# DredderGun/accbpg_and_fw

Measured on AMD Instinct MI355X. Metric: D-opt iters/sec (m=2048,n=32768), higher is better.
Workload: dtype f64; 1 GPU; D_opt_design(2048,32768) abpg_gain gamma=2 fp64, one independent instance per GPU; instances=1, instances_per_gpu=1, seeds=1..1, window=transient: iterations 5..161 from x0 = 1/n, linear_gram=False

## Files before the change

### accbpg_and_fw_amd/csrc/dopt_kernels.hip

```cpp
#include <atomic>
#include <mutex>
#include <unordered_map>
#include <type_traits>

#include "internal.h"
#include "mfma_tile.hpp"

namespace accbpg {

struct GramSeg {
    int64_t row0, col0, kb, ke;
    bool dual, whole;
};
constexpr int GRAM_RMAX = 4;
template <class T>
__device__ __forceinline__ GramSeg gram_segment(const TileRC* __restrict__ tiles, int64_t kiters, int64_t it,
                                                int64_t it1) {
    const int e = (int)(it / kiters);
    const int64_t off = it - (int64_t)e * kiters;
    const TileRC tr = tiles[e];
    GramSeg g;
    if (tr.d1 < 0) {
        g.row0 = (int64_t)tr.rb * T::BM; g.col0 = (int64_t)tr.cb * T::BN;
        g.kb = off; g.ke = min(kiters, off + (it1 - it));
// ... 390 lines not shown
    const int64_t col0 = (int64_t)blockIdx.x * T::BN;
    const int lane = threadIdx.x & 63, wave = __builtin_amdgcn_readfirstlane(threadIdx.x >> 6);
    const int wm = wave / T::WAVES_N, wn = wave % T::WAVES_N;
    const int lr = lane & 15;
    double colsum[T::NI];
#pragma unroll
    for (int j = 0; j < T::NI; ++j) colsum[j] = 0.0;
    T t;
    const int nrb = (int)((m + T::BM - 1) / T::BM);
    for (int rb = 0; rb < nrb; ++rb) {
        const int64_t row0 = (int64_t)rb * T::BM;
        const int64_t Kend = min(row0 + T::BM, m);
        const int64_t ksteps = (Kend + BK - 1) / BK;
        t.zero();
        t.gload_A(W, ldw, row0, m, 0, Kend, vec_ok_w);
        t.gload_B_km(V, ldv, col0, n, 0, Kend, vec_ok_v);
        __syncthreads();
        t.sstore(lds);
        __syncthreads();
        const int64_t klast = ksteps - 1;
        {
            const int64_t k1 = min((int64_t)1, klast);
            t.gload_A(W, ldw, row0, m, k1 * BK, Kend, vec_ok_w);
            t.gload_B_km(V, ldv, col0, n, k1 * BK, Kend, vec_ok_v);
        }
        t.template read_frag<0>(lds, 0);
        int cur = 0;
#pragma unroll 1
        for (int64_t ks = 0; ks < ksteps; ++ks) {
            const int64_t k2 = min(ks + 2, klast);
            const double* st = lds + cur * T::STAGE_ELEMS;
            double* nx = lds + (cur ^ 1) * T::STAGE_ELEMS;
            const int64_t kd = ks * BK - row0;
            int mi_lo = 0;
            if (kd > 0) {
                const int64_t num = kd - 15 - 16 * wm;
                mi_lo = num > 0 ? (int)((num + 16 * T::WAVES_M - 1) / (16 * T::WAVES_M)) : 0;
            }
            t.template read_frag<1>(st, 1);
            t.template mma_frag<0>(mi_lo);
            t.template read_frag<0>(st, 2);
            t.template mma_frag<1>(mi_lo);
            t.template read_frag<1>(st, 3);
            t.sstore(nx);
            t.template mma_frag<0>(mi_lo);
            __syncthreads();
            t.gload_A(W, ldw, row0, m, k2 * BK, Kend, vec_ok_w);
            t.gload_B_km(V, ldv, col0, n, k2 * BK, Kend, vec_ok_v);
            t.template read_frag<0>(nx, 0);
            t.template mma_frag<1>(mi_lo);
            cur ^= 1;
        }
#pragma unroll
        for (int j = 0; j < T::NI; ++j) {
            double s = 0.0;
#pragma unroll
            for (int i = 0; i < T::MI; ++i)
#pragma unroll
                for (int r = 0; r < 4; ++r) s += t.acc[i][j][r] * t.acc[i][j][r];
            colsum[j] += s;
        }
    }
#pragma unroll
    for (int j = 0; j < T::NI; ++j) {
        double s = colsum[j];
        s += __shfl_xor(s, 16);
        s += __shfl_xor(s, 32);
        colsum[j] = s;
    }
    if (lane < 16) {
#pragma unroll
        for (int j = 0; j < T::NI; ++j) red[wm][wn * T::WN + 16 * j + lr] = colsum[j];
    }
    __syncthreads();
    for (int c = threadIdx.x; c < T::BN; c += NTHREADS) {
        double s = 0.0;
#pragma unroll
        for (int w = 0; w < T::WAVES_M; ++w) s += red[w][c];
        if (col0 + c < n) out[col0 + c] = sign * s;
    }
}

constexpr int COLNORM_CV = 256;

template <class T, int G, int JJ, int RUN, int NLD>
__device__ __forceinline__ void colnorm_diag_step(T& t, double* __restrict__ lds, int& cur, int wm, int64_t kdiag,
                                                  int64_t ldv, const char* next_a) {
    int nx1 = cur + 1;
    if (nx1 >= 3) nx1 -= 3;
    int nx2 = cur + 2;
    if (nx2 >= 3) nx2 -= 3;
    constexpr int J = 4 * G + JJ;
    int64_t k2 = kdiag + J + 2;
    if constexpr (J >= 14) {
        if constexpr (J == 14) t.gbase_a = next_a;
        k2 = J - 14;
    }
    constexpr int ILO_NEXT = JJ == 3 ? ((G + 1) & 3) : G;
    t.template grad_step<RUN, G, ILO_NEXT, (JJ > 0), NLD>(lds + cur * T::G_STAGE, lds + nx1 * T::G_STAGE, lds + nx2 * T::G_STAGE,
                                                          k2 * BK, k2 * BK * ldv, wm >= JJ);
    cur = nx1;
}
template <class T, int G, int RUN, int NLD>
__device__ __forceinline__ void colnorm_diag_group(T& t, double* __restrict__ lds, int& cur, int wm, int64_t kdiag,
                                                   int64_t ldv, const char* next_a) {
    colnorm_diag_step<T, G, 0, RUN, NLD>(t, lds, cur, wm, kdiag, ldv, next_a);
    colnorm_diag_step<T, G, 1, RUN, NLD>(t, lds, cur, wm, kdiag, ldv, next_a);
    colnorm_diag_step<T, G, 2, RUN, NLD>(t, lds, cur, wm, kdiag, ldv, next_a);
    colnorm_diag_step<T, G, 3, RUN, NLD>(t, lds, cur, wm, kdiag, ldv, next_a);
}

template <class T>
__device__ __forceinline__ void colnorm_phases_body(
    const double* __restrict__ W, int64_t ldw, const double* __restrict__ V, int64_t ldv, int64_t m, int64_t n,
    double* __restrict__ out, double sign) {
    extern __shared__ __attribute__((aligned(16))) double lds[];
    double* red = lds + 3 * T::G_STAGE;
    constexpr int NLD = T::G_NA + T::G_NB;
    constexpr int RUN = 4;
    static_assert(T::WAVES_N == 1 && T::MI == 4 && T::BM == 16 * BK, "diagonal groups are laid out for the 256 x 128 tile");
    const int64_t col0 = (int64_t)blockIdx.x * T::BN;
    const int lane = threadIdx.x & 63, wave = __builtin_amdgcn_readfirstlane(threadIdx.x >> 6);
    const int wm = wave / T::WAVES_N, wn = wave % T::WAVES_N;
    const int lr = lane & 15;
    double colsum[T::NI];
#pragma unroll
    for (int j = 0; j < T::NI; ++j) colsum[j] = 0.0;
    T t;
    const int nrb = (int)(m / T::BM);
    t.template glds_setup_A<RUN>(W, ldw, 0);
    t.template glds_setup_B_km<RUN>(V, ldv, col0);
    t.template glds_issue<RUN>(0, 0, lds);
    t.template glds_issue<RUN>(BK, BK * ldv, lds + T::G_STAGE);
    asm volatile("s_waitcnt vmcnt(%0)" ::"n"(NLD) : "memory");
    __builtin_amdgcn_s_barrier();
    int cur = 0;
    t.template read_frag_lo<0, 0>(lds, 0);
    t.zero();
    t.pin_acc();
    for (int rb = 0;;) {
        const int64_t kdiag = (int64_t)rb * (T::BM / BK);
        const int rbn = rb + 1 < nrb ? rb + 1 : rb;
        const char* next_a = reinterpret_cast<const char*>(W + (int64_t)rbn * T::BM * ldw);
        colnorm_diag_group<T, 0, RUN, NLD>(t, lds, cur, wm, kdiag, ldv, next_a);
        colnorm_diag_group<T, 1, RUN, NLD>(t, lds, cur, wm, kdiag, ldv, next_a);
        colnorm_diag_group<T, 2, RUN, NLD>(t, lds, cur, wm, kdiag, ldv, next_a);
        colnorm_diag_group<T, 3, RUN, NLD>(t, lds, cur, wm, kdiag, ldv, next_a);
#pragma unroll
        for (int j = 0; j < T::NI; ++j) {
            t.pin_acc_col(j);
            double s = 0.0;
#pragma unroll
            for (int i = 0; i < T::MI; ++i)
#pragma unroll
                for (int r = 0; r < 4; ++r) s += t.acc[i][j][r] * t.acc[i][j][r];
            colsum[j] += s;
            asm volatile("" : "+v"(colsum[j]));
            __builtin_amdgcn_sched_barrier(0);
        }
        if (++rb == nrb) break;
        t.zero();
        t.pin_acc();
        const int64_t krect = (int64_t)rb * (T::BM / BK);
        int64_t ks = 0;
#pragma unroll 1
        do {
            int nx1 = cur + 1;
            if (nx1 >= 3) nx1 -= 3;
            int nx2 = cur + 2;
            if (nx2 >= 3) nx2 -= 3;
            const int64_t k2 = (ks + 2) * BK;
            t.template grad_step<RUN, 0, 0, false, NLD>(lds + cur * T::G_STAGE, lds + nx1 * T::G_STAGE, lds + nx2 * T::G_STAGE,
                                                        k2, k2 * ldv, true);
            cur = nx1;
        } while (++ks < krect);
    }
    asm volatile("s_waitcnt vmcnt(0)\n\ts_waitcnt lgkmcnt(0)" ::: "memory");
#pragma unroll
    for (int j = 0; j < T::NI; ++j) {
        double s = colsum[j];
        s += __shfl_xor(s, 16);
        s += __shfl_xor(s, 32);
        colsum[j] = s;
    }
    __syncthreads();
    if (lane < 16) {
#pragma unroll
        for (int j = 0; j < T::NI; ++j) red[wm * T::BN + wn * T::WN + 16 * j + lr] = colsum[j];
    }
    __syncthreads();
    for (int c = threadIdx.x; c < T::BN; c += NTHREADS) {
        double s = 0.0;
#pragma unroll
        for (int w = 0; w < T::WAVES_M; ++w) s += red[w * T::BN + c];
        if (col0 + c < n) out[col0 + c] = sign * s;
    }
}

template <class T, int CV>
__device__ __forceinline__ void colnorm_restart_body(
    const double* __restrict__ W, int64_t ldw, const double* __restrict__ V, int64_t ldv, int64_t m, int64_t n,
    double* __restrict__ out, double sign) {
    constexpr int AB = (CV & 512) ? (CV & 15) : 0;
    extern __shared__ __attribute__((aligned(16))) double lds[];
    double* red = lds + 3 * T::G_STAGE;
    constexpr int NLD = T::G_NA + T::G_NB;
    const int64_t col0 = (int64_t)blockIdx.x * T::BN;
    const int lane = threadIdx.x & 63, wave = __builtin_amdgcn_readfirstlane(threadIdx.x >> 6);
    const int wm = wave / T::WAVES_N, wn = wave % T::WAVES_N;
    const int lr = lane & 15;
    double colsum[T::NI];
#pragma unroll
    for (int j = 0; j < T::NI; ++j) colsum[j] = 0.0;
    T t;
    const int nrb = (int)(m / T::BM);
    for (int rb = 0; rb < nrb; ++rb) {
        const int64_t row0 = (int64_t)rb * T::BM;
        const int64_t ksteps = (row0 + T::BM) / BK;
        const int64_t klast = ksteps - 1;
        t.zero();
        constexpr int RUN = (CV & 256) ? 4 : 1;
        t.template glds_setup_A<RUN>(W, ldw, row0);
        t.template glds_setup_B_km<RUN>(V, ldv, col0);
        auto issue = [&](int64_t ks, int buf) {
            t.template glds_issue<RUN>(ks * BK, ks * BK * ldv, lds + buf * T::G_STAGE);
        };
        const int64_t ks0 = (AB & 2) ? row0 / BK : 0, ks1 = (AB & 1) ? row0 / BK : ksteps;
        if (!(AB & 8) || rb == 0) {
            __builtin_amdgcn_s_barrier();
            issue(ks0, 0);
            issue(min(ks0 + 1, klast), 1);
            asm volatile("s_waitcnt vmcnt(%0)" ::"n"(NLD) : "memory");
            __builtin_amdgcn_s_barrier();
        }
        int cur = 0;
        t.template read_frag_g<0, false>(lds, 0);
        if constexpr (CV & 32) {
            constexpr int NP = T::G_NA + T::G_NB;
#pragma unroll 1
            for (int64_t ks = ks0; ks < ks1; ++ks) {
                int nx2 = cur + 2;
                if (nx2 >= 3) nx2 -= 3;
                int nx1 = cur + 1;
                if (nx1 >= 3) nx1 -= 3;
                const double* st = lds + cur * T::G_STAGE;
                const double* st1 = lds + nx1 * T::G_STAGE;
                double* nst = lds + nx2 * T::G_STAGE;
                const int64_t kd = ks * BK - row0;
                int mi_lo = 0;
                if (kd > 0) {
                    const int64_t num = kd - 15 - 16 * wm;
                    mi_lo = num > 0 ? (int)((num + 16 * T::WAVES_M - 1) / (16 * T::WAVES_M)) : 0;
                }
                const int64_t k2 = min(ks + 2, klast) * BK;
                auto group = [&](auto gtag) {
                    constexpr int g = decltype(gtag)::value;
// ... 33 lines not shown
            }
        } else {
#pragma unroll 1
        for (int64_t ks = ks0; ks < ks1; ++ks) {
            int nx2 = cur + 2;
            if (nx2 >= 3) nx2 -= 3;
            const double* st = lds + cur * T::G_STAGE;
            const int64_t kd = ks * BK - row0;
            int mi_lo = 0;
            if (kd > 0) {
                const int64_t num = kd - 15 - 16 * wm;
                mi_lo = num > 0 ? (int)((num + 16 * T::WAVES_M - 1) / (16 * T::WAVES_M)) : 0;
            }
            constexpr int NP = T::G_NA + T::G_NB;
            constexpr int P1 = (NP + 2) / 3, P2 = 2 * P1 < NP ? 2 * P1 : NP;
            static_assert(T::MI == 4, "group 0 is dealt out over four fragment rows");
            double* nst = lds + nx2 * T::G_STAGE;
            const int64_t k2 = min(ks + 2, klast) * BK;
            if constexpr (!(AB & 4)) t.template read_frag_g<1, false>(st, 1);
            __builtin_amdgcn_sched_barrier(0);
            t.template mma_row<0>(0, mi_lo);
            if constexpr (!(AB & 4)) t.template glds_issue_range<RUN>(k2, k2 * ldv, nst, 0, P1);
            t.template mma_row<0>(1, mi_lo);
            if constexpr (!(AB & 4)) t.template glds_issue_range<RUN>(k2, k2 * ldv, nst, P1, P2);
            t.template mma_row<0>(2, mi_lo);
            if constexpr (!(AB & 4)) t.template glds_issue_range<RUN>(k2, k2 * ldv, nst, P2, NP);
            t.template mma_row<0>(3, mi_lo);
            __builtin_amdgcn_sched_barrier(0);
            if constexpr (!(AB & 4)) t.template read_frag_g<0, false>(st, 2);
            __builtin_amdgcn_sched_barrier(0);
            t.template mma_frag<1>(mi_lo);
            __builtin_amdgcn_sched_barrier(0);
            if constexpr (!(AB & 4)) t.template read_frag_g<1, false>(st, 3);
            __builtin_amdgcn_sched_barrier(0);
            t.template mma_frag<0>(mi_lo);
            __builtin_amdgcn_sched_barrier(0);
            if constexpr (!(AB & 4)) {
                asm volatile("s_waitcnt vmcnt(%0)\n\ts_waitcnt lgkmcnt(0)" ::"n"(NLD) : "memory");
                __builtin_amdgcn_s_barrier();
            }
            cur = (cur + 1 == 3) ? 0 : cur + 1;
            if constexpr (!(AB & 4)) t.template read_frag_g<0, false>(lds + cur * T::G_STAGE, 0);
            __builtin_amdgcn_sched_barrier(0);
            t.template mma_frag<1>(mi_lo);
            __builtin_amdgcn_sched_barrier(0);
        }
        }
        if (!(AB & 8) || rb == nrb - 1) asm volatile("s_waitcnt vmcnt(0)\n\ts_waitcnt lgkmcnt(0)" ::: "memory");
#pragma unroll
        for (int j = 0; j < T::NI; ++j) {
            double s = 0.0;
#pragma unroll
            for (int i = 0; i < T::MI; ++i)
#pragma unroll
                for (int r = 0; r < 4; ++r) s += t.acc[i][j][r] * t.acc[i][j][r];
            colsum[j] += s;
        }
    }
#pragma unroll
    for (int j = 0; j < T::NI; ++j) {
        double s = colsum[j];
        s += __shfl_xor(s, 16);
        s += __shfl_xor(s, 32);
        colsum[j] = s;
    }
    __syncthreads();
    if (lane < 16) {
#pragma unroll
        for (int j = 0; j < T::NI; ++j) red[wm * T::BN + wn * T::WN + 16 * j + lr] = colsum[j];
    }
    __syncthreads();
    for (int c = threadIdx.x; c < T::BN; c += NTHREADS) {
        double s = 0.0;
#pragma unroll
        for (int w = 0; w < T::WAVES_M; ++w) s += red[w * T::BN + c];
        if (col0 + c < n) out[col0 + c] = sign * s;
    }
}

template <class T, int CV = 0>
__device__ __forceinline__ void colnorm_glds_body(
    const double* __restrict__ W, int64_t ldw, const double* __restrict__ V, int64_t ldv, int64_t m, int64_t n,
    double* __restrict__ out, double sign) {
    if constexpr (CV == COLNORM_CV) colnorm_phases_body<T>(W, ldw, V, ldv, m, n, out, sign);
    else colnorm_restart_body<T, CV>(W, ldw, V, ldv, m, n, out, sign);
}

template <class T, int CV = 0>
__global__ __launch_bounds__(NTHREADS, 1) void colnorm_glds_kernel(
    const double* __restrict__ W, int64_t ldw, const double* __restrict__ V, int64_t ldv, int64_t m, int64_t n,
    double* __restrict__ out, double sign) {
    colnorm_glds_body<T, CV>(W, ldw, V, ldv, m, n, out, sign);
}
template <class T>
__global__ __launch_bounds__(NTHREADS, 1) void colnorm_glds_batch_kernel(
    const BatchInst* __restrict__ bt, BatchAct act, int64_t ldw, int64_t ldv, int64_t m, int64_t n,
    double* __restrict__ outbase, int64_t ldo, double sign) {
    const int inst = act.idx[blockIdx.y];
    const BatchInst bi = bt[inst];
    colnorm_glds_body<T, COLNORM_CV>(bi.Wbuf, ldw, bi.V, ldv, m, n, outbase + (int64_t)inst * ldo, sign);
}

template <class T, int LOOP>
__device__ __forceinline__ void gemm_ops_body(const GemmOp op) {
    extern __shared__ __attribute__((aligned(16))) double lds[];
    const int64_t row0 = (int64_t)blockIdx.y * T::BM, col0 = (int64_t)blockIdx.x * T::BN;
    if (row0 >= op.M || col0 >= op.N) return;
    if (op.lower_only && col0 > row0 + T::BM - 1) return;
    const bool va = ((reinterpret_cast<uintptr_t>(op.A) & 15) == 0) && ((op.lda & 1) == 0);
    const bool vb = ((reinterpret_cast<uintptr_t>(op.B) & 15) == 0) && ((op.ldb & 1) == 0);
    T t;
    t.zero();
    int64_t ksteps = (op.K + BK - 1) / BK;
    int64_t ks0 = 0;
    if (op.tri & 1) ks0 = max((int64_t)0, col0 - op.koff) / BK;
    if (op.tri & 2) ksteps = min(ksteps, max((int64_t)0, row0 + T::BM - op.koff + BK - 1) / BK);
    if (ks0 >= ksteps) {
        t.store_C(op.C, op.ldc, row0, col0, op.M, op.N, op.alpha, op.beta, op.lower_only != 0);
        return;
    }
    if constexpr (LOOP == 0) {
        auto gload = [&](int64_t ks) {
            t.gload_A(op.A, op.lda, row0, op.M, ks * BK, op.K, va);
            if constexpr (T::BKM) t.gload_B_km(op.B, op.ldb, col0, op.N, ks * BK, op.K, vb);
            else t.gload_B_kc(op.B, op.ldb, col0, op.N, ks * BK, op.K, vb);
        };
        gload(ks0);
        t.sstore(lds);
        __syncthreads();
        int cur = 0;
        for (int64_t ks = ks0; ks < ksteps; ++ks) {
            const bool more = ks + 1 < ksteps;
            if (more) gload(ks + 1);
            t.compute(lds + cur * T::STAGE_ELEMS);
            if (more) t.sstore(lds + (cur ^ 1) * T::STAGE_ELEMS);
            __syncthreads();
            cur ^= 1;
        }
    } else {
        constexpr int D = LOOP;
        const bool inside = va && vb && row0 + T::BM <= op.M && col0 + T::BN <= op.N && ksteps * BK <= op.K;
        d2 pa[D][T::A_PASS], pb[D][T::B_PASS];
        auto sstore_from = [&](auto slot, double* __restrict__ stage) {
            constexpr int S = decltype(slot)::value;
#pragma unroll
            for (int p = 0; p < T::A_PASS; ++p) t.ra[p] = pa[S][p];
#pragma unroll
            for (int p = 0; p < T::B_PASS; ++p) t.rb[p] = pb[S][p];
            t.sstore(stage);
        };
        auto run = [&](auto guard) {
            constexpr bool GUARD = decltype(guard)::value;
            auto gload_to = [&](auto slot, int64_t ks) {
                constexpr int S = decltype(slot)::value;
                t.template gload_A<GUARD>(as_global(op.A), op.lda, row0, op.M, ks * BK, op.K, va);
                if constexpr (T::BKM) t.template gload_B_km<GUARD>(as_global(op.B), op.ldb, col0, op.N, ks * BK, op.K, vb);
                else t.template gload_B_kc<GUARD>(as_global(op.B), op.ldb, col0, op.N, ks * BK, op.K, vb);
#pragma unroll
                for (int p = 0; p < T::A_PASS; ++p) pa[S][p] = t.ra[p];
#pragma unroll
                for (int p = 0; p < T::B_PASS; ++p) pb[S][p] = t.rb[p];
            };
            static_for<0, D>([&](auto j) {
                if (ks0 + decltype(j)::value < ksteps) gload_to(j, ks0 + decltype(j)::value);
            });
            sstore_from(std::integral_constant<int, 0>{}, lds);
            if (ks0 + D < ksteps) gload_to(std::integral_constant<int, 0>{}, ks0 + D);
// ... 1843 lines not shown
    accbpg_dopt* h0 = b->inst[0];
    static bool lds_set = false;
    if (!lds_set) {
        ACC_TRY(set_lds(gram_streamk_glds_batch_kernel<T>, T::G_LDS_BYTES));
        lds_set = true;
    }
    prof_begin(h0, PROF_GRAM);
    gram_streamk_glds_batch_kernel<T><<<dim3(h0->gram_grid, act.n), NTHREADS, T::G_LDS_BYTES, b->stream>>>(
        b->table, act, h0->ldv, h0->m, h0->n, xbase, ldx, h0->tiles, h0->wg_ranges, h0->kiters, h0->gram_nslot, h0->m);
    prof_end(h0, PROF_GRAM);
    prof_begin(h0, PROF_GRAMFIX);
    gram_fixup_batch_kernel<T><<<dim3(h0->ntiles * 2 * T::MI * FIX_PJ, act.n), NTHREADS, 0, b->stream>>>(
        b->table, act, h0->tiles, h0->gram_cstart, h0->gram_contrib, h0->gram_nslot, h0->m, h0->m);
    prof_end(h0, PROF_GRAMFIX);
    ACC_HIP(hipGetLastError());
    return ACCBPG_OK;
}

int launch_cholesky_batch(accbpg_dopt_batch* b, const BatchAct& act, bool with_inverse, const double* xbase, int64_t ldx) {
    accbpg_dopt* h0 = b->inst[0];
    const int64_t m = h0->m;
    const int T = (int)((m + NB - 1) / NB);
    prof_begin(h0, PROF_CHOL);
    zero_scalars_batch_kernel<<<act.n, 512, 0, b->stream>>>(b->table, act, xbase, ldx, h0->n, T * T + 5 * T);
    const int dev = (b->device >= 0 && b->device < 64) ? b->device : 0;
    const int grid_all = h0->chol_tiles_grid * act.n;
    std::lock_guard<std::mutex> lk(g_tiles_mu);
    TilesRing& ring = g_tiles[dev];
    {
        int gmax = grid_all;
        for (int i = 0; i < TILES_RING; ++i) gmax = std::max(gmax, ring.grid[i]);
        int together = std::max(1, h0->chol_slots) / std::max(1, gmax);
        if (together > TILES_RING - 1) together = TILES_RING - 1;
        if (together < 1) together = 1;
        for (long long back = together; back <= TILES_RING && back <= ring.issued; ++back) {
            const int slot = (int)((ring.issued - back) % TILES_RING);
            if (ring.ev[slot] && ring.stream[slot] != b->stream) ACC_HIP(hipStreamWaitEvent(b->stream, ring.ev[slot], 0));
        }
    }
    chol_tiles_kernel<<<dim3(h0->chol_tiles_grid, act.n), NTHREADS, CT_LDS_BYTES, b->stream>>>(
        CholInst{}, b->chol_table[with_inverse ? 1 : 0], reinterpret_cast<const CholJob*>(h0->chol_jobs), m, m, T,
        h0->chol_spin_limit, 0, act);
    prof_end(h0, PROF_CHOL);
    ACC_HIP(hipGetLastError());
    {
        const int slot = (int)(ring.issued % TILES_RING);
        if (!ring.ev[slot]) ACC_HIP(hipEventCreateWithFlags(&ring.ev[slot], hipEventDisableTiming));
        ACC_HIP(hipEventRecord(ring.ev[slot], b->stream));
        ring.stream[slot] = b->stream;
        ring.grid[slot] = grid_all;
        ++ring.issued;
    }
    return ACCBPG_OK;
}

int launch_trtri_batch(accbpg_dopt_batch* b, const BatchAct& act) {
    accbpg_dopt* h0 = b->inst[0];
    prof_begin(h0, PROF_TRTRI);
    for (const accbpg_dopt::MergeStage& st : h0->merge_stages) {
        const int count = st.end - st.begin;
        if (count <= 0) continue;
        if (st.kind == 0) {
            dim3 grid((st.maxn + 63) / 64, (st.maxm + 63) / 64, count * act.n);
            ACC_TRY(with_gemm_loop([&](auto loop) -> int {
                gemm_ops_batch_kernel<TileSmall<true>, decltype(loop)::value><<<grid, NTHREADS, TileSmall<true>::LDS_BYTES, b->stream>>>(
                    b->ops_all, b->ops_per_inst, st.begin, count, act);
                return ACCBPG_OK;
            }));
        } else {
            int gx = (int)std::min<int64_t>(1024, ((int64_t)st.maxm / 2 + 255) / 256);
            gemm_reduce_batch_kernel<<<dim3(gx, count * act.n), 256, 0, b->stream>>>(b->red_all, b->red_per_inst, st.begin, count, act);
        }
    }
    prof_end(h0, PROF_TRTRI);
    ACC_HIP(hipGetLastError());
    return ACCBPG_OK;
}

int debug_grad_variant(accbpg_dopt* h, double* out, int var, int iters, double* ms_out) {
    using T = TileBig<true, false>;
    const bool vw = ((reinterpret_cast<uintptr_t>(h->Wbuf) & 15) == 0) && ((h->m & 1) == 0);
    if (!h->big || !h->use_glds || !vw || !h->vec_ok || h->m % 256 != 0 || h->n % 128 != 0) return ACCBPG_ERR_ARG;
    const int grid = (int)(h->n / T::BN), lds = T::G_LDS_BYTES + 4 * T::BN * 8;
    if (var != 0 && var != 3 && (var < 10 || var > 13)) return ACCBPG_ERR_ARG;
    hipEvent_t a, b;
    ACC_HIP(hipEventCreate(&a));
    if (hipEventCreate(&b) != hipSuccess) {
        hipEventDestroy(a);
        return ACCBPG_ERR_HIP;
    }
    auto launch = [&]() -> int {
#define ACC_LAUNCH_C(CC) \
    ACC_LAUNCH_LDS((colnorm_glds_kernel<T, CC>), grid, NTHREADS, lds, h->stream, h->Wbuf, h->m, h->V, h->ldv, h->m, h->n, out, -1.0)
        switch (var) {
            case 0: ACC_LAUNCH_C(COLNORM_CV); break;
            case 3: ACC_LAUNCH_C(COLNORM_CV | 512); break;
            case 10: ACC_LAUNCH_C(COLNORM_CV | 512 | 1); break;
            case 11: ACC_LAUNCH_C(COLNORM_CV | 512 | 2); break;
            case 12: ACC_LAUNCH_C(COLNORM_CV | 512 | 4); break;
            case 13: ACC_LAUNCH_C(COLNORM_CV | 512 | 8); break;
            default: return ACCBPG_ERR_ARG;
        }
#undef ACC_LAUNCH_C
        return ACCBPG_OK;
    };
    auto timed = [&]() -> int {
        ACC_TRY(launch());
        ACC_HIP(hipEventRecord(a, h->stream));
        for (int i = 0; i < iters; ++i) ACC_TRY(launch());
        ACC_HIP(hipEventRecord(b, h->stream));
        ACC_HIP(hipEventSynchronize(b));
        float ms = 0.f;
        ACC_HIP(hipEventElapsedTime(&ms, a, b));
        *ms_out = ms / iters;
        ACC_HIP(hipGetLastError());
        return ACCBPG_OK;
    };
    const int rc = timed();
    hipEventDestroy(a);
    hipEventDestroy(b);
    return rc;
}

int launch_colnorm_batch(accbpg_dopt_batch* b, const BatchAct& act, double* gbase, int64_t ldg, double sign) {
    using T = TileBig<true, false>;
    accbpg_dopt* h0 = b->inst[0];
    static bool lds_set = false;
    if (!lds_set) {
        ACC_TRY(set_lds(colnorm_glds_batch_kernel<T>, T::G_LDS_BYTES + 4 * T::BN * 8));
        lds_set = true;
    }
    prof_begin(h0, PROF_GRAD);
    colnorm_glds_batch_kernel<T><<<dim3((unsigned)(h0->n / T::BN), act.n), NTHREADS, T::G_LDS_BYTES + 4 * T::BN * 8, b->stream>>>(
        b->table, act, h0->m, h0->ldv, h0->m, h0->n, gbase, ldg, sign);
    prof_end(h0, PROF_GRAD);
    ACC_HIP(hipGetLastError());
    return ACCBPG_OK;
}

int launch_test_gemm(const double* A, int64_t lda, const double* B, int64_t ldb, double* C, int64_t ldc, int64_t M,
                     int64_t N, int64_t K, int b_kmajor, double alpha, double beta, int config, hipStream_t s) {
    GemmOp op{};
    op.A = A; op.B = B; op.C = C; op.lda = lda; op.ldb = ldb; op.ldc = ldc;
    op.M = (int)M; op.N = (int)N; op.K = (int)K; op.lower_only = 0; op.alpha = alpha; op.beta = beta;
    if (config == 1) {
        if (b_kmajor) {
            using T = TileBig<true>;
            ACC_TRY(set_lds(gemm_big_kernel<T>, T::LDS_BYTES));
            dim3 grid((unsigned)((N + T::BN - 1) / T::BN), (unsigned)((M + T::BM - 1) / T::BM));
            gemm_big_kernel<T><<<grid, NTHREADS, T::LDS_BYTES, s>>>(op);
        } else {
            using T = TileBig<false>;
            ACC_TRY(set_lds(gemm_big_kernel<T>, T::LDS_BYTES));
            dim3 grid((unsigned)((N + T::BN - 1) / T::BN), (unsigned)((M + T::BM - 1) / T::BM));
            gemm_big_kernel<T><<<grid, NTHREADS, T::LDS_BYTES, s>>>(op);
        }
    } else {
        GemmOp* d = nullptr;
        ACC_HIP(hipMalloc(&d, sizeof(GemmOp)));
        ACC_HIP(hipMemcpyAsync(d, &op, sizeof(GemmOp), hipMemcpyHostToDevice, s));
        ACC_TRY(set_lds_gemm_ops());
        int rc = launch_gemm_ops(d, 1, (int)M, (int)N, b_kmajor != 0, s);
        hipStreamSynchronize(s);
        hipFree(d);
        return rc;
    }
    ACC_HIP(hipGetLastError());
    return ACCBPG_OK;
}

int pipe_probe(int iters, int mode, double* ms_out, hipStream_t s) {
    int dev = 0;
    hipDeviceProp_t prop;
    ACC_HIP(hipGetDevice(&dev));
    ACC_HIP(hipGetDeviceProperties(&prop, dev));
    double* sink = nullptr;
    ACC_HIP(hipMalloc(&sink, 8));
    hipEvent_t a, b;
    ACC_HIP(hipEventCreate(&a));
    ACC_HIP(hipEventCreate(&b));
    pipe_probe_kernel<<<prop.multiProcessorCount, NTHREADS, 0, s>>>(iters / 10 + 1, mode, sink);
    ACC_HIP(hipEventRecord(a, s));
    pipe_probe_kernel<<<prop.multiProcessorCount, NTHREADS, 0, s>>>(iters, mode, sink);
// ... 37 lines not shown
```

### accbpg_and_fw_amd/csrc/mfma_tile.hpp

```cpp
#pragma once
#include <hip/hip_runtime.h>
#include <stdint.h>
#include <type_traits>

namespace accbpg {

typedef double d4 __attribute__((ext_vector_type(4)));
typedef double d2 __attribute__((ext_vector_type(2)));

constexpr int BK = 16;
constexpr int SK = BK + 2;
constexpr int NTHREADS = 256;

typedef const __attribute__((address_space(1))) double* gptr;
__device__ __forceinline__ gptr as_global(const double* p) { return (gptr)p; }
__device__ __forceinline__ d2 ld2(const double* p) { return *reinterpret_cast<const d2*>(p); }
__device__ __forceinline__ d2 ld2(gptr p) { return *(const __attribute__((address_space(1))) d2*)p; }

template <class P>
__device__ __forceinline__ d2 load2_guard(P p, bool row_ok, int64_t k, int64_t K, bool vec_ok) {
    d2 v;
    if (row_ok && vec_ok && k + 1 < K) {
        v = ld2(p);
    } else {
// ... 352 lines not shown
        if constexpr (BKM) {
            const double* bs = stage + G_A + (4 * kk + lq) * BN + wn * WN + lr;
#pragma unroll
            for (int j = 0; j < NI; ++j) fb[SET][j] = bs[16 * (j ^ (lq & 1))];
        } else {
            const double* bs = stage + G_A + (wn * WN + lr) * BK + koff;
#pragma unroll
            for (int j = 0; j < NI; ++j) fb[SET][j] = bs[j * 16 * BK];
        }
        if constexpr (SCALE) fx[SET] = stage[G_A + G_B + 4 * kk + lq];
    }

    template <int SET, bool SCALE, int PART>
    __device__ __forceinline__ void read_part_g(const double* __restrict__ stage, int kk) {
        static_assert(MI == 4 && NI == 8, "parts are laid out for the 64 x 128 wave tile");
        const int lane = threadIdx.x & 63, wave = __builtin_amdgcn_readfirstlane(threadIdx.x >> 6);
        const int wm = wave / WAVES_N, wn = wave % WAVES_N;
        const int lr = lane & 15, lq = lane >> 4;
        const int sw = (lr >> 1) & 7;
        const int koff = 2 * ((2 * kk + (lq >> 1)) ^ sw) + (lq & 1);
        if constexpr (PART == 0) {
            if constexpr (SCALE) fx[SET] = stage[G_A + G_B + 4 * kk + lq];
        } else if constexpr (PART == 1 || PART == 6) {
            const double* as = stage + (16 * wm + lr) * BK + koff;
            constexpr int i0 = (PART == 1) ? 0 : 2;
            fa[SET][i0] = as[i0 * 16 * WAVES_M * BK];
            fa[SET][i0 + 1] = as[(i0 + 1) * 16 * WAVES_M * BK];
        } else {
            constexpr int j0 = 2 * (PART - 2);
            if constexpr (BKM) {
                const double* bs = stage + G_A + (4 * kk + lq) * BN + wn * WN + lr;
                fb[SET][j0] = bs[16 * (j0 ^ (lq & 1))];
                fb[SET][j0 + 1] = bs[16 * ((j0 + 1) ^ (lq & 1))];
            } else {
                const double* bs = stage + G_A + (wn * WN + lr) * BK + koff;
                fb[SET][j0] = bs[j0 * 16 * BK];
                fb[SET][j0 + 1] = bs[(j0 + 1) * 16 * BK];
            }
        }
    }
    template <int SET, int I>
    __device__ __forceinline__ void scale_row() { fa[SET][I] *= fx[SET]; }
    template <int SET, int I, int P>
    __device__ __forceinline__ void mma_pair(int mi_lo = 0) {
        if (I >= mi_lo) {
            acc[I][2 * P] = __builtin_amdgcn_mfma_f64_16x16x4f64(fa[SET][I], fb[SET][2 * P], acc[I][2 * P], 0, 0, 0);
            acc[I][2 * P + 1] = __builtin_amdgcn_mfma_f64_16x16x4f64(fa[SET][I], fb[SET][2 * P + 1], acc[I][2 * P + 1], 0, 0, 0);
        }
    }

    template <int SET, int ILO>
    __device__ __forceinline__ void read_frag_lo(const double* __restrict__ stage, int kk) {
        static_assert(BKM, "the gradient product reads a k-major B image");
        const int lane = threadIdx.x & 63, wave = __builtin_amdgcn_readfirstlane(threadIdx.x >> 6);
        const int wm = wave / WAVES_N, wn = wave % WAVES_N;
        const int lr = lane & 15, lq = lane >> 4;
        const int sw = (lr >> 1) & 7;
        const int koff = 2 * ((2 * kk + (lq >> 1)) ^ sw) + (lq & 1);
        const double* as = stage + (16 * wm + lr) * BK + koff;
#pragma unroll
        for (int i = ILO; i < MI; ++i) fa[SET][i] = as[i * 16 * WAVES_M * BK];
        const double* bs = stage + G_A + (4 * kk + lq) * BN + wn * WN + lr;
#pragma unroll
        for (int j = 0; j < NI; ++j) fb[SET][j] = bs[16 * (j ^ (lq & 1))];
    }
    template <int SET, int I, int ILO, bool COND>
    __device__ __forceinline__ void mma_row_lo(bool live) {
        if constexpr (I >= ILO) {
            if (!(COND && I == ILO) || live) {
#pragma unroll
                for (int j = 0; j < NI; ++j)
                    acc[I][j] = __builtin_amdgcn_mfma_f64_16x16x4f64(fa[SET][I], fb[SET][j], acc[I][j], 0, 0, 0);
            }
        }
    }
    template <int SET, int ILO, bool COND>
    __device__ __forceinline__ void mma_frag_lo(bool live) {
        static_assert(MI == 4, "four fragment rows");
        mma_row_lo<SET, 0, ILO, COND>(live);
        mma_row_lo<SET, 1, ILO, COND>(live);
        mma_row_lo<SET, 2, ILO, COND>(live);
        mma_row_lo<SET, 3, ILO, COND>(live);
    }
    template <int RUN, int ILO, int ILO_NEXT, bool COND, int NLD>
    __device__ __forceinline__ void grad_step(const double* __restrict__ st, const double* __restrict__ st1,
                                              double* __restrict__ nst, int64_t ka, int64_t kb, bool live) {
        constexpr int NP = G_NA + G_NB;
        constexpr int P1 = (NP + 2) / 3, P2 = 2 * P1 < NP ? 2 * P1 : NP;
        static_assert(NLD == NP, "every wave retires the loads of one step per step");
        read_frag_lo<1, ILO>(st, 1);
        __builtin_amdgcn_sched_barrier(0);
        mma_row_lo<0, 0, ILO, COND>(live);
        glds_issue_range<RUN>(ka, kb, nst, 0, P1);
        mma_row_lo<0, 1, ILO, COND>(live);
        glds_issue_range<RUN>(ka, kb, nst, P1, P2);
        mma_row_lo<0, 2, ILO, COND>(live);
        glds_issue_range<RUN>(ka, kb, nst, P2, NP);
        mma_row_lo<0, 3, ILO, COND>(live);
        __builtin_amdgcn_sched_barrier(0);
        read_frag_lo<0, ILO>(st, 2);
        __builtin_amdgcn_sched_barrier(0);
        mma_frag_lo<1, ILO, COND>(live);
        __builtin_amdgcn_sched_barrier(0);
        read_frag_lo<1, ILO>(st, 3);
        __builtin_amdgcn_sched_barrier(0);
        mma_frag_lo<0, ILO, COND>(live);
        __builtin_amdgcn_sched_barrier(0);
        asm volatile("s_waitcnt vmcnt(%0)\n\ts_waitcnt lgkmcnt(0)" ::"n"(NLD) : "memory");
        __builtin_amdgcn_s_barrier();
        read_frag_lo<0, ILO_NEXT>(st1, 0);
        __builtin_amdgcn_sched_barrier(0);
        mma_frag_lo<1, ILO, COND>(live);
        __builtin_amdgcn_sched_barrier(0);
    }

    double fb2[2][NI];
    __device__ __forceinline__ void glds_setup_A_dual(const double* __restrict__ V, int64_t ldv, int64_t band0,
                                                      int64_t khalf) {
        const int lane = threadIdx.x & 63, wave = __builtin_amdgcn_readfirstlane(threadIdx.x >> 6);
        gbase_a = reinterpret_cast<const char*>(V + band0 * ldv);
#pragma unroll
        for (int p = 0; p < G_NA; ++p) {
            const int q = wave + 4 * p;
            const int row = 8 * q + (lane >> 3);
            const int c = (lane & 7) ^ ((row >> 1) & 7);
            goa[p] = (uint32_t)(((int64_t)(row & (BM / 2 - 1)) * ldv + 2 * c + ((row >= BM / 2) ? khalf : 0)) * 8);
        }
    }
    __device__ __forceinline__ void glds_issue_dual(int64_t ka, const double* __restrict__ x, int64_t khalf,
                                                    double* __restrict__ stage) const {
        const int lane = threadIdx.x & 63, wave = __builtin_amdgcn_readfirstlane(threadIdx.x >> 6);
        const char* ba = gbase_a + ka * 8;
#pragma unroll
        for (int p = 0; p < G_NA; ++p) {
            uint32_t o = goa[p];
            asm volatile("" : "+v"(o));
            glds16(reinterpret_cast<const double*>(ba + o), stage + (wave + 4 * p) * 128);
        }
        const float* sx = reinterpret_cast<const float*>(x + ka + ((lane & 32) ? khalf : 0)) + (lane & 31);
        __builtin_amdgcn_global_load_lds((const __attribute__((address_space(1))) void*)sx,
                                         (__attribute__((address_space(3))) void*)(stage + G_A + G_B), 4, 0, 0);
    }
    static constexpr int G_NLD_DUAL = G_NA + 1;
    static __device__ __forceinline__ int dual_row_block(int i2, int w) {
        return i2 ? (2 * WAVES_M - 1 - w) : w;
    }
    template <int SET>
    __device__ __forceinline__ void read_frag_dual(const double* __restrict__ stage, int kk) {
        const int lane = threadIdx.x & 63, wave = __builtin_amdgcn_readfirstlane(threadIdx.x >> 6);
        const int lr = lane & 15, lq = lane >> 4;
        const int sw = (lr >> 1) & 7;
        const int koff = 2 * ((2 * kk + (lq >> 1)) ^ sw) + (lq & 1);
#pragma unroll
        for (int i = 0; i < MI; ++i)
            fa[SET][i] = stage[((i / (MI / 2)) * (BM / 2) + 16 * dual_row_block(i % (MI / 2), wave) + lr) * BK + koff];
        const double* bs = stage + lr * BK + koff;
#pragma unroll
        for (int j = 0; j < NI; ++j) {
            fb[SET][j] = bs[j * 16 * BK];
            fb2[SET][j] = bs[(BM / 2 + j * 16) * BK];
        }
        fx[SET] = stage[G_A + G_B + 4 * kk + lq];
        fx2[SET] = stage[G_A + G_B + 16 + 4 * kk + lq];
    }
    double fx2[2];
    template <int SET>
    __device__ __forceinline__ void scale_dual() {
#pragma unroll
        for (int i = 0; i < MI; ++i) fa[SET][i] *= (i < MI / 2) ? fx[SET] : fx2[SET];
    }
    template <int SET>
    __device__ __forceinline__ void mma_dual() {
        const int wave = __builtin_amdgcn_readfirstlane(threadIdx.x >> 6);
#pragma unroll
        for (int i = 0; i < MI; ++i) {
            const int lim = dual_row_block(i % (MI / 2), wave);
#pragma unroll
            for (int j = 0; j < NI; ++j) {
                if (j > lim) break;
                acc[i][j] = __builtin_amdgcn_mfma_f64_16x16x4f64(fa[SET][i], (i < MI / 2) ? fb[SET][j] : fb2[SET][j],
                                                                 acc[i][j], 0, 0, 0);
            }
        }
    }
    __device__ __forceinline__ void store_C(double* __restrict__ C, int64_t ldc, int64_t row0, int64_t col0,
                                            int64_t M, int64_t N, double alpha, double beta, bool lower_only) const {
        const int lane = threadIdx.x & 63, wave = __builtin_amdgcn_readfirstlane(threadIdx.x >> 6);
        const int wm = wave / WAVES_N, wn = wave % WAVES_N;
        const int lr = lane & 15, lq = lane >> 4;
#pragma unroll
        for (int i = 0; i < MI; ++i)
#pragma unroll
            for (int j = 0; j < NI; ++j)
#pragma unroll
                for (int r = 0; r < 4; ++r) {
                    const int64_t row = row0 + 16 * (i * WAVES_M + wm) + lq + 4 * r;
// ... 133 lines not shown
```

Before: 64.49 iterations/s.

## Interleave fragment reads and global loads between individual MFMA pairs in colnorm

```diff
diff --git a/accbpg_and_fw_amd/csrc/dopt_kernels.hip b/accbpg_and_fw_amd/csrc/dopt_kernels.hip
--- a/accbpg_and_fw_amd/csrc/dopt_kernels.hip
+++ b/accbpg_and_fw_amd/csrc/dopt_kernels.hip
@@ -496,8 +496,11 @@
 }
 
 constexpr int COLNORM_CV = 256;
-
-template <class T, int G, int JJ, int RUN, int NLD>
+constexpr int COLNORM_BLOCK = 1024, COLNORM_OTHER_PLACEMENT = 2048, COLNORM_ABLATE = 4096, COLNORM_DIAG_BLOCK = 8192;
+constexpr bool COLNORM_PB = true;
+constexpr bool colnorm_pb(int cv) { return ((cv & COLNORM_OTHER_PLACEMENT) != 0) != COLNORM_PB; }
+
+template <class T, int G, int JJ, int RUN, int NLD, int CV>
 __device__ __forceinline__ void colnorm_diag_step(T& t, double* __restrict__ lds, int& cur, int wm, int64_t kdiag,
                                                   int64_t ldv, const char* next_a) {
     int nx1 = cur + 1;
@@ -511,20 +514,25 @@
         k2 = J - 14;
     }
     constexpr int ILO_NEXT = JJ == 3 ? ((G + 1) & 3) : G;
-    t.template grad_step<RUN, G, ILO_NEXT, (JJ > 0), NLD>(lds + cur * T::G_STAGE, lds + nx1 * T::G_STAGE, lds + nx2 * T::G_STAGE,
-                                                          k2 * BK, k2 * BK * ldv, wm >= JJ);
+    constexpr int AB = (CV & COLNORM_ABLATE) ? (CV & 7) : 0;
+    if constexpr (!(CV & (COLNORM_BLOCK | COLNORM_DIAG_BLOCK)) && T::template dealt_pairs_per_group<G, (JJ > 0)>() >= 12)
+        t.template grad_step_dealt<RUN, G, ILO_NEXT, (JJ > 0), NLD, colnorm_pb(CV), AB>(
+            lds + cur * T::G_STAGE, lds + nx1 * T::G_STAGE, lds + nx2 * T::G_STAGE, k2 * BK, k2 * BK * ldv, wm >= JJ);
+    else
+        t.template grad_step<RUN, G, ILO_NEXT, (JJ > 0), NLD, AB>(lds + cur * T::G_STAGE, lds + nx1 * T::G_STAGE, lds + nx2 * T::G_STAGE,
+                                                                  k2 * BK, k2 * BK * ldv, wm >= JJ);
     cur = nx1;
 }
-template <class T, int G, int RUN, int NLD>
+template <class T, int G, int RUN, int NLD, int CV>
 __device__ __forceinline__ void colnorm_diag_group(T& t, double* __restrict__ lds, int& cur, int wm, int64_t kdiag,
                                                    int64_t ldv, const char* next_a) {
-    colnorm_diag_step<T, G, 0, RUN, NLD>(t, lds, cur, wm, kdiag, ldv, next_a);
-    colnorm_diag_step<T, G, 1, RUN, NLD>(t, lds, cur, wm, kdiag, ldv, next_a);
-    colnorm_diag_step<T, G, 2, RUN, NLD>(t, lds, cur, wm, kdiag, ldv, next_a);
-    colnorm_diag_step<T, G, 3, RUN, NLD>(t, lds, cur, wm, kdiag, ldv, next_a);
-}
-
-template <class T>
+    colnorm_diag_step<T, G, 0, RUN, NLD, CV>(t, lds, cur, wm, kdiag, ldv, next_a);
+    colnorm_diag_step<T, G, 1, RUN, NLD, CV>(t, lds, cur, wm, kdiag, ldv, next_a);
+    colnorm_diag_step<T, G, 2, RUN, NLD, CV>(t, lds, cur, wm, kdiag, ldv, next_a);
+    colnorm_diag_step<T, G, 3, RUN, NLD, CV>(t, lds, cur, wm, kdiag, ldv, next_a);
+}
+
+template <class T, int CV>
 __device__ __forceinline__ void colnorm_phases_body(
     const double* __restrict__ W, int64_t ldw, const double* __restrict__ V, int64_t ldv, int64_t m, int64_t n,
     double* __restrict__ out, double sign) {
@@ -532,6 +540,8 @@
     double* red = lds + 3 * T::G_STAGE;
     constexpr int NLD = T::G_NA + T::G_NB;
     constexpr int RUN = 4;
+    constexpr int AB = (CV & COLNORM_ABLATE) ? (CV & 7) : 0;
+    constexpr bool PB = colnorm_pb(CV);
     static_assert(T::WAVES_N == 1 && T::MI == 4 && T::BM == 16 * BK, "diagonal groups are laid out for the 256 x 128 tile");
     const int64_t col0 = (int64_t)blockIdx.x * T::BN;
     const int lane = threadIdx.x & 63, wave = __builtin_amdgcn_readfirstlane(threadIdx.x >> 6);
@@ -550,16 +560,17 @@
     __builtin_amdgcn_s_barrier();
     int cur = 0;
     t.template read_frag_lo<0, 0>(lds, 0);
+    if constexpr (AB & 4) t.template read_frag_lo<1, 0>(lds, 1);
     t.zero();
     t.pin_acc();
     for (int rb = 0;;) {
         const int64_t kdiag = (int64_t)rb * (T::BM / BK);
         const int rbn = rb + 1 < nrb ? rb + 1 : rb;
         const char* next_a = reinterpret_cast<const char*>(W + (int64_t)rbn * T::BM * ldw);
-        colnorm_diag_group<T, 0, RUN, NLD>(t, lds, cur, wm, kdiag, ldv, next_a);
-        colnorm_diag_group<T, 1, RUN, NLD>(t, lds, cur, wm, kdiag, ldv, next_a);
-        colnorm_diag_group<T, 2, RUN, NLD>(t, lds, cur, wm, kdiag, ldv, next_a);
-        colnorm_diag_group<T, 3, RUN, NLD>(t, lds, cur, wm, kdiag, ldv, next_a);
+        colnorm_diag_group<T, 0, RUN, NLD, CV>(t, lds, cur, wm, kdiag, ldv, next_a);
+        colnorm_diag_group<T, 1, RUN, NLD, CV>(t, lds, cur, wm, kdiag, ldv, next_a);
+        colnorm_diag_group<T, 2, RUN, NLD, CV>(t, lds, cur, wm, kdiag, ldv, next_a);
+        colnorm_diag_group<T, 3, RUN, NLD, CV>(t, lds, cur, wm, kdiag, ldv, next_a);
 #pragma unroll
         for (int j = 0; j < T::NI; ++j) {
             t.pin_acc_col(j);
@@ -584,8 +595,12 @@
             int nx2 = cur + 2;
             if (nx2 >= 3) nx2 -= 3;
             const int64_t k2 = (ks + 2) * BK;
-            t.template grad_step<RUN, 0, 0, false, NLD>(lds + cur * T::G_STAGE, lds + nx1 * T::G_STAGE, lds + nx2 * T::G_STAGE,
-                                                        k2, k2 * ldv, true);
+            if constexpr (CV & COLNORM_BLOCK)
+                t.template grad_step<RUN, 0, 0, false, NLD, AB>(lds + cur * T::G_STAGE, lds + nx1 * T::G_STAGE, lds + nx2 * T::G_STAGE,
+                                                                k2, k2 * ldv, true);
+            else
+                t.template grad_step_dealt<RUN, 0, 0, false, NLD, PB, AB>(lds + cur * T::G_STAGE, lds + nx1 * T::G_STAGE,
+                                                                          lds + nx2 * T::G_STAGE, k2, k2 * ldv, true);
             cur = nx1;
         } while (++ks < krect);
     }
@@ -785,7 +800,7 @@
 __device__ __forceinline__ void colnorm_glds_body(
     const double* __restrict__ W, int64_t ldw, const double* __restrict__ V, int64_t ldv, int64_t m, int64_t n,
     double* __restrict__ out, double sign) {
-    if constexpr (CV == COLNORM_CV) colnorm_phases_body<T>(W, ldw, V, ldv, m, n, out, sign);
+    if constexpr ((CV & 256) && !(CV & 512)) colnorm_phases_body<T, CV>(W, ldw, V, ldv, m, n, out, sign);
     else colnorm_restart_body<T, CV>(W, ldw, V, ldv, m, n, out, sign);
 }
 
@@ -2795,7 +2810,7 @@
     const bool vw = ((reinterpret_cast<uintptr_t>(h->Wbuf) & 15) == 0) && ((h->m & 1) == 0);
     if (!h->big || !h->use_glds || !vw || !h->vec_ok || h->m % 256 != 0 || h->n % 128 != 0) return ACCBPG_ERR_ARG;
     const int grid = (int)(h->n / T::BN), lds = T::G_LDS_BYTES + 4 * T::BN * 8;
-    if (var != 0 && var != 3 && (var < 10 || var > 13)) return ACCBPG_ERR_ARG;
+    if (var != 0 && (var < 3 || var > 6) && (var < 10 || var > 13) && (var < 20 || var > 23) && (var < 30 || var > 33)) return ACCBPG_ERR_ARG;
     hipEvent_t a, b;
     ACC_HIP(hipEventCreate(&a));
     if (hipEventCreate(&b) != hipSuccess) {
@@ -2812,6 +2827,17 @@
             case 11: ACC_LAUNCH_C(COLNORM_CV | 512 | 2); break;
             case 12: ACC_LAUNCH_C(COLNORM_CV | 512 | 4); break;
             case 13: ACC_LAUNCH_C(COLNORM_CV | 512 | 8); break;
+            case 4: ACC_LAUNCH_C(COLNORM_CV | COLNORM_BLOCK); break;
+            case 5: ACC_LAUNCH_C(COLNORM_CV | COLNORM_OTHER_PLACEMENT); break;
+            case 6: ACC_LAUNCH_C(COLNORM_CV | COLNORM_DIAG_BLOCK); break;
+            case 20: ACC_LAUNCH_C(COLNORM_CV | COLNORM_BLOCK | COLNORM_ABLATE | 7); break;
+            case 21: ACC_LAUNCH_C(COLNORM_CV | COLNORM_BLOCK | COLNORM_ABLATE | 6); break;
+            case 22: ACC_LAUNCH_C(COLNORM_CV | COLNORM_BLOCK | COLNORM_ABLATE | 3); break;
+            case 23: ACC_LAUNCH_C(COLNORM_CV | COLNORM_BLOCK | COLNORM_ABLATE | 2); break;
+            case 30: ACC_LAUNCH_C(COLNORM_CV | COLNORM_ABLATE | 7); break;
+            case 31: ACC_LAUNCH_C(COLNORM_CV | COLNORM_ABLATE | 6); break;
+            case 32: ACC_LAUNCH_C(COLNORM_CV | COLNORM_ABLATE | 3); break;
+            case 33: ACC_LAUNCH_C(COLNORM_CV | COLNORM_ABLATE | 2); break;
             default: return ACCBPG_ERR_ARG;
         }
 #undef ACC_LAUNCH_C
diff --git a/accbpg_and_fw_amd/csrc/mfma_tile.hpp b/accbpg_and_fw_amd/csrc/mfma_tile.hpp
--- a/accbpg_and_fw_amd/csrc/mfma_tile.hpp
+++ b/accbpg_and_fw_amd/csrc/mfma_tile.hpp
@@ -458,36 +458,110 @@
         mma_row_lo<SET, 2, ILO, COND>(live);
         mma_row_lo<SET, 3, ILO, COND>(live);
     }
-    template <int RUN, int ILO, int ILO_NEXT, bool COND, int NLD>
+    template <int RUN, int ILO, int ILO_NEXT, bool COND, int NLD, int AB = 0>
     __device__ __forceinline__ void grad_step(const double* __restrict__ st, const double* __restrict__ st1,
                                               double* __restrict__ nst, int64_t ka, int64_t kb, bool live) {
         constexpr int NP = G_NA + G_NB;
         constexpr int P1 = (NP + 2) / 3, P2 = 2 * P1 < NP ? 2 * P1 : NP;
         static_assert(NLD == NP, "every wave retires the loads of one step per step");
-        read_frag_lo<1, ILO>(st, 1);
+        if constexpr (!(AB & 4)) read_frag_lo<1, ILO>(st, 1);
         __builtin_amdgcn_sched_barrier(0);
         mma_row_lo<0, 0, ILO, COND>(live);
-        glds_issue_range<RUN>(ka, kb, nst, 0, P1);
+        if constexpr (!(AB & 1)) glds_issue_range<RUN>(ka, kb, nst, 0, P1);
         mma_row_lo<0, 1, ILO, COND>(live);
-        glds_issue_range<RUN>(ka, kb, nst, P1, P2);
+        if constexpr (!(AB & 1)) glds_issue_range<RUN>(ka, kb, nst, P1, P2);
         mma_row_lo<0, 2, ILO, COND>(live);
-        glds_issue_range<RUN>(ka, kb, nst, P2, NP);
+        if constexpr (!(AB & 1)) glds_issue_range<RUN>(ka, kb, nst, P2, NP);
         mma_row_lo<0, 3, ILO, COND>(live);
         __builtin_amdgcn_sched_barrier(0);
-        read_frag_lo<0, ILO>(st, 2);
+        if constexpr (!(AB & 4)) read_frag_lo<0, ILO>(st, 2);
         __builtin_amdgcn_sched_barrier(0);
         mma_frag_lo<1, ILO, COND>(live);
         __builtin_amdgcn_sched_barrier(0);
-        read_frag_lo<1, ILO>(st, 3);
+        if constexpr (!(AB & 4)) read_frag_lo<1, ILO>(st, 3);
         __builtin_amdgcn_sched_barrier(0);
         mma_frag_lo<0, ILO, COND>(live);
         __builtin_amdgcn_sched_barrier(0);
-        asm volatile("s_waitcnt vmcnt(%0)\n\ts_waitcnt lgkmcnt(0)" ::"n"(NLD) : "memory");
-        __builtin_amdgcn_s_barrier();
-        read_frag_lo<0, ILO_NEXT>(st1, 0);
+        if constexpr (!(AB & 2)) {
+            asm volatile("s_waitcnt vmcnt(%0)\n\ts_waitcnt lgkmcnt(0)" ::"n"(NLD) : "memory");
+            __builtin_amdgcn_s_barrier();
+        }
+        if constexpr (!(AB & 4)) read_frag_lo<0, ILO_NEXT>(st1, 0);
         __builtin_amdgcn_sched_barrier(0);
         mma_frag_lo<1, ILO, COND>(live);
         __builtin_amdgcn_sched_barrier(0);
+    }
+
+    static constexpr int DEALT_PART_VALUES = 2;
+    template <int SET, int PART, int ILO>
+    __device__ __forceinline__ void read_part_lo(const double* __restrict__ stage, int kk) {
+        if constexpr (PART == 1 || PART == 6) {
+            const int lane = threadIdx.x & 63, wave = __builtin_amdgcn_readfirstlane(threadIdx.x >> 6);
+            const int wm = wave / WAVES_N;
+            const int lr = lane & 15, lq = lane >> 4;
+            const int sw = (lr >> 1) & 7;
+            const int koff = 2 * ((2 * kk + (lq >> 1)) ^ sw) + (lq & 1);
+            const double* as = stage + (16 * wm + lr) * BK + koff;
+            constexpr int i0 = (PART == 1) ? 0 : 2;
+            if constexpr (i0 >= ILO) fa[SET][i0] = as[i0 * 16 * WAVES_M * BK];
+            if constexpr (i0 + 1 >= ILO) fa[SET][i0 + 1] = as[(i0 + 1) * 16 * WAVES_M * BK];
+        } else {
+            read_part_g<SET, false, PART>(stage, kk);
+        }
+    }
+    template <int RUN, int ILO, int ILO_NEXT, int NU, bool PB, int AB, int G, int U>
+    __device__ __forceinline__ void dealt_behind(const double* __restrict__ st, const double* __restrict__ st1,
+                                                 double* __restrict__ nst, int64_t ka, int64_t kb) {
+        constexpr int NP = G_NA + G_NB;
+        constexpr int QBAR = PB ? NU / 4 : NU / 2;
+        if constexpr (G < 3) {
+            constexpr int rp = PB ? U + (NU == 16 ? 0 : 1) : (((U & 1) == 1) ? (U >> 1) + 1 : -1);
+            if constexpr (rp >= 1 && rp < 7 && !(AB & 4)) read_part_lo<(G & 1) ^ 1, (rp >= 1 && rp < 7) ? rp : 1, ILO>(st, G + 1);
+            constexpr int lp = PB ? U - NU / 2 : (((U & 1) == 0) ? (U >> 1) : -1);
+            if constexpr (G == 0 && lp >= 0 && 2 * lp < NP && (2 * lp) % RUN == 0 && !(AB & 1))
+                glds_issue_range<RUN>(ka, kb, nst, 2 * lp, 2 * lp + RUN);
+        } else {
+            constexpr int rp = U - QBAR + 1;
+            if constexpr (rp >= 1 && rp < 7 && !(AB & 4)) read_part_lo<0, (rp >= 1 && rp < 7) ? rp : 1, ILO_NEXT>(st1, 0);
+        }
+    }
+    template <int RUN, int ILO, int ILO_NEXT, int NU, bool PB, int AB, int NLD, int G, int U>
+    __device__ __forceinline__ void dealt_pairs(const double* __restrict__ st, const double* __restrict__ st1,
+                                                double* __restrict__ nst, int64_t ka, int64_t kb) {
+        if constexpr (U < NU) {
+            if constexpr (G == 3 && U == (PB ? NU / 4 : NU / 2) && !(AB & 2)) {
+                asm volatile("s_waitcnt vmcnt(%0)\n\ts_waitcnt lgkmcnt(0)" ::"n"(NLD) : "memory");
+                __builtin_amdgcn_s_barrier();
+            }
+            mma_pair<(G & 1), (MI - NU / 4 + U / 4), (U % 4)>();
+            __builtin_amdgcn_sched_barrier(0);
+            dealt_behind<RUN, ILO, ILO_NEXT, NU, PB, AB, G, U>(st, st1, nst, ka, kb);
+            __builtin_amdgcn_sched_barrier(0);
+            dealt_pairs<RUN, ILO, ILO_NEXT, NU, PB, AB, NLD, G, U + 1>(st, st1, nst, ka, kb);
+        }
+    }
+    template <int ILO, bool COND>
+    static constexpr int dealt_pairs_per_group() { return 4 * (MI - ILO - (COND ? 1 : 0)); }
+    template <int RUN, int ILO, int ILO_NEXT, bool COND, int NLD, bool PB, int AB = 0>
+    __device__ __forceinline__ void grad_step_dealt(const double* __restrict__ st, const double* __restrict__ st1,
+                                                    double* __restrict__ nst, int64_t ka, int64_t kb, bool live) {
+        constexpr int NU = dealt_pairs_per_group<ILO, COND>();
+        static_assert(MI == 4 && NI == 8 && BKM, "pairs and parts are laid out for the 64 x 128 wave tile, k-major B");
+        static_assert(NLD == G_NA + G_NB && (G_NA + G_NB) % RUN == 0 && RUN % 2 == 0, "every wave retires the loads of one step per step, in whole runs");
+        static_assert(NU >= 12 && (G_NA + G_NB) / 2 <= 6, "one thing behind a pair: six read parts, and the loads behind the second half of group 0");
+        __builtin_amdgcn_sched_barrier(0);
+        mma_row_lo<0, ILO, COND ? ILO : MI, COND>(live);
+        __builtin_amdgcn_sched_barrier(0);
+        dealt_pairs<RUN, ILO, ILO_NEXT, NU, PB, AB, NLD, 0, 0>(st, st1, nst, ka, kb);
+        mma_row_lo<1, ILO, COND ? ILO : MI, COND>(live);
+        __builtin_amdgcn_sched_barrier(0);
+        dealt_pairs<RUN, ILO, ILO_NEXT, NU, PB, AB, NLD, 1, 0>(st, st1, nst, ka, kb);
+        mma_row_lo<0, ILO, COND ? ILO : MI, COND>(live);
+        __builtin_amdgcn_sched_barrier(0);
+        dealt_pairs<RUN, ILO, ILO_NEXT, NU, PB, AB, NLD, 2, 0>(st, st1, nst, ka, kb);
+        mma_row_lo<1, ILO, COND ? ILO : MI, COND>(live);
+        __builtin_amdgcn_sched_barrier(0);
+        dealt_pairs<RUN, ILO, ILO_NEXT, NU, PB, AB, NLD, 3, 0>(st, st1, nst, ka, kb);
     }
 
     double fb2[2][NI];
```

After: 65.55 iterations/s, median of 6. +1.7%, better.
